# Dhole/collaborative_filtering

Measured on AMD Instinct MI355X. Metric: user-subgraph eigendecomps/sec + predicted ratings/sec, 1M users avg deg 100, higher is better.
Workload: dtype f32 (eigen) / f64 (predict)

## Files before the change

### collaborative_filtering_amd/_native.py

```python
from __future__ import annotations

import ctypes
import os
from ctypes import POINTER, c_char_p, c_double, c_float, c_int, c_int32, c_uint32, c_uint64, c_void_p

_HERE = os.path.dirname(os.path.abspath(__file__))
LIB_PATH = os.environ.get("CF_MI355X_LIB") or os.path.join(_HERE, "libcf_mi355x.so")
HOST_LIB_PATH = os.path.join(_HERE, "libcf_host.so")

CF_OK = 0
CF_EINVAL = -1
CF_ERANGE = -4
CF_ESTATE = -5
CF_KNN_SCORE_SUM = 0
CF_KNN_SCORE_MEAN = 1
CF_SVD_MAX_NV = 256
CF_ALS_MAX_D = 64
CF_TOPN_MAX_N = 1024
CF_SIGS_OWN = 0
CF_SIGS_COMPAT = 1
CF_MAX_K = 192
CF_SPILL_MAX_K = 5000
CF_EIGEN_TRIDIAG = 0
CF_EIGEN_JACOBI = 1
CF_GRAPH_DENSE = 0
CF_GRAPH_CSR = 1
CF_FILTER_CHEBY = 0
CF_FILTER_BINOMIAL = 1

SIGNATURES = {
    "cf_version": (c_int, []),
    "cf_device_count": (c_int, []),
    "cf_create": (c_int, [c_int, POINTER(c_void_p)]),
    "cf_destroy": (None, [c_void_p]),
    "cf_release_workspaces": (c_int, [c_void_p]),
    "cf_last_error": (c_char_p, [c_void_p]),
    "cf_set_jacobi": (c_int, [c_void_p, c_float, c_int]),
    "cf_set_eigen_refine": (c_int, [c_void_p, c_int, c_float, c_float]),
    "cf_set_eigen_split": (c_int, [c_void_p, c_int]),
    "cf_set_eigen_lanes": (c_int, [c_void_p, c_int]),
    "cf_debug_eigen_geometry": (c_int, [c_int, c_int, POINTER(c_int), POINTER(c_int), POINTER(c_int), POINTER(c_int),
                                        POINTER(c_int)]),
    "cf_set_pred_pack": (c_int, [c_void_p, c_int]),
    "cf_debug_split_schedule": (c_int, [c_int, c_int, POINTER(c_int), POINTER(c_int), POINTER(c_int), POINTER(c_int)]),
    "cf_set_step_masks": (c_int, [c_void_p, c_int]),
    "cf_set_local_wlim": (c_int, [c_void_p, c_int]),
    "cf_debug_predict_nmax": (c_int, [c_int]),
    "cf_set_knn2_topk": (c_int, [c_void_p, c_uint32]),
    "cf_set_eigen_method": (c_int, [c_void_p, c_int]),
    "cf_debug_stats": (c_int, [c_void_p, c_int, c_void_p]),
    "cf_eigen_bucket_timing": (c_int, [c_void_p, c_int, c_void_p]),
    "cf_eigen_bucket_timing_split": (c_int, [c_void_p, c_int, c_void_p, c_void_p]),
    "cf_debug_phases": (c_int, [c_void_p, c_int, c_void_p]),
    "cf_debug_spill": (c_int, [c_void_p, c_int, c_void_p]),
    "cf_debug_tri": (c_int, [c_void_p, c_int, c_void_p]),
    "cf_item_graph_upload": (c_int, [c_void_p, c_uint32, c_void_p, c_void_p, c_void_p]),
    "cf_item_graph_upload_dense": (c_int, [c_void_p, c_uint32, c_void_p, c_int]),
    "cf_item_graph_device": (c_void_p, [c_void_p, POINTER(c_uint32)]),
    "cf_set_graph_layout": (c_int, [c_void_p, c_int]),
    "cf_graph_info": (c_int, [c_void_p, c_void_p, c_void_p, c_void_p]),
    "cf_item_cosine_edges": (c_int, [c_void_p, c_uint32, c_uint32, c_void_p, c_void_p, c_void_p, c_float, c_int, c_int,
                                     c_void_p, c_void_p, c_void_p, c_uint64, c_void_p]),
    "cf_plan_create": (c_int, [c_void_p, c_uint32, c_void_p, POINTER(c_void_p)]),
    "cf_plan_destroy": (None, [c_void_p]),
    "cf_evec_slots": (c_uint64, [c_uint32]),
    "cf_evec_offsets": (c_uint64, [c_uint32, c_void_p, c_void_p]),
# ... 211 lines not shown
```

### collaborative_filtering_amd/api.py

```python
from __future__ import annotations

from ctypes import byref, c_double, c_float, c_int, c_uint32, c_void_p
from dataclasses import dataclass

import numpy as np

from . import _native
from ._native import CF_ERANGE, CF_FILTER_BINOMIAL, CF_FILTER_CHEBY, CF_SIGS_COMPAT, CF_SIGS_OWN, NativeError, ptr


def _check(lib, ctx, rc, what):
    if rc != _native.CF_OK:
        msg = lib.cf_last_error(ctx)
        raise NativeError(f"{what} failed ({rc}): {msg.decode() if msg else ''}")


def evec_offsets(item_off: np.ndarray) -> tuple[np.ndarray, int]:
    k = np.diff(item_off.astype(np.int64))
    slots = k * np.maximum(k, 2)
    off = np.zeros(len(k), dtype=np.uint64)
    if len(k):
        off[1:] = np.cumsum(slots)[:-1]
    return off, int(slots.sum())

# ... 279 lines not shown
            pass

    def _chk(self, rc, what):
        _check(self.lib, self.h, rc, what)

    def set_eigen_method(self, method: str = "jacobi"):
        code = {"tridiag": _native.CF_EIGEN_TRIDIAG, "jacobi": _native.CF_EIGEN_JACOBI}[method]
        self._chk(self.lib.cf_set_eigen_method(self.h, code), "cf_set_eigen_method")

    def set_jacobi(self, tol_scale: float = 1.0, max_sweeps: int = 30):
        self._chk(self.lib.cf_set_jacobi(self.h, tol_scale, max_sweeps), "cf_set_jacobi")

    def set_eigen_refine(self, enable: bool = True, stop_rel: float = 1e-3, delta: float = 1e-2):
        self._chk(self.lib.cf_set_eigen_refine(self.h, int(enable), stop_rel, delta), "cf_set_eigen_refine")

    def set_eigen_split(self, enable=True):
        self._chk(self.lib.cf_set_eigen_split(self.h, int(enable)), "cf_set_eigen_split")

    def set_eigen_lanes(self, lanes=0):
        self._chk(self.lib.cf_set_eigen_lanes(self.h, int(lanes)), "cf_set_eigen_lanes")

    def set_pred_pack(self, mode=1):
        self._chk(self.lib.cf_set_pred_pack(self.h, int(mode)), "cf_set_pred_pack")

    def set_local_wlim(self, bisect: bool = True):
        self._chk(self.lib.cf_set_local_wlim(self.h, int(bisect)), "cf_set_local_wlim")

    def set_step_masks(self, enable: bool = True):
        self._chk(self.lib.cf_set_step_masks(self.h, int(enable)), "cf_set_step_masks")

    def debug_stats(self, enable: bool = True, read: bool = False):
        out = np.zeros(8, dtype=np.uint64) if read else None
        self._chk(self.lib.cf_debug_stats(self.h, int(enable), ptr(out)), "cf_debug_stats")
        if read:
            n = max(int(out[1]), 1)
            return {"sweeps_mean": int(out[0]) / n, "users": int(out[1]), "sweeps_max": int(out[2]),
                    "capped": int(out[3]), "assembly_cyc_per_user": int(out[4]) / n,
                    "jacobi_cyc_per_user": int(out[5]) / n, "epilogue_cyc_per_user": int(out[6]) / n,
                    "jacobi_cyc_per_step": int(out[5]) / max(int(out[7]), 1)}
        return None

    def eigen_bucket_timing(self, enable: bool = True, read: bool = False, sweeps: bool = False):
        out = np.zeros(13, dtype=np.float32) if read else None
        sw = np.zeros(13, dtype=np.float32) if read else None
        self._chk(self.lib.cf_eigen_bucket_timing_split(self.h, int(enable), ptr(out), ptr(sw)),
                  "cf_eigen_bucket_timing_split")
# ... 852 lines not shown
```

### collaborative_filtering_amd/csrc/cf_api.hip

```cpp

#include <algorithm>
#include <atomic>
#include <cmath>
#include <cstring>
#include <new>

#include <type_traits>

#include "cf_internal.h"

int cf_set_error(cf_ctx* ctx, int code, const std::string& msg) {
    if (ctx) ctx->last_error = msg;
    return code;
}

namespace {
constexpr int kMaxDevices = 64;
std::atomic<int> g_ctx_per_device[kMaxDevices];
}

int cf_contexts_on_device(int device) {
    return (device >= 0 && device < kMaxDevices) ? g_ctx_per_device[device].load() : 1;
}

// ... 103 lines not shown
    drop(ctx->d_tri, ctx->tri_bytes);
    drop(ctx->d_scratch, ctx->scratch_bytes);
    drop(ctx->d_knn, ctx->knn_bytes);
    drop(ctx->d_als, ctx->als_bytes);
    return CF_OK;
}

void cf_destroy(cf_ctx* ctx) {
    if (!ctx) return;
    g_ctx_per_device[ctx->device].fetch_sub(1);
    (void)hipSetDevice(ctx->device);
    if (ctx->d_graph) (void)hipFree(ctx->d_graph);
    if (ctx->d_grp) (void)hipFree(ctx->d_grp);
    if (ctx->d_gcol) (void)hipFree(ctx->d_gcol);
    if (ctx->d_gw) (void)hipFree(ctx->d_gw);
    cf_knn_in_free(ctx);
    if (ctx->d_stats) (void)hipFree(ctx->d_stats);
    if (ctx->d_dbg) (void)hipFree(ctx->d_dbg);
    if (ctx->d_phase) (void)hipFree(ctx->d_phase);
    if (ctx->d_scratch) (void)hipFree(ctx->d_scratch);
    if (ctx->d_pred_next) (void)hipFree(ctx->d_pred_next);
    if (ctx->d_dense_q) (void)hipFree(ctx->d_dense_q);
    if (ctx->d_dense_ws) (void)hipFree(ctx->d_dense_ws);
    if (ctx->d_cmask) (void)hipFree(ctx->d_cmask);
    if (ctx->d_cmask_fp) (void)hipFree(ctx->d_cmask_fp);
    if (ctx->d_knn) (void)hipFree(ctx->d_knn);
    if (ctx->d_knn_acc) (void)hipFree(ctx->d_knn_acc);
    if (ctx->d_knn_part) (void)hipFree(ctx->d_knn_part);
    if (ctx->d_prep) (void)hipFree(ctx->d_prep);
    if (ctx->d_als) (void)hipFree(ctx->d_als);
    for (hipEvent_t& e : ctx->prep_ev)
        if (e) (void)hipEventDestroy(e);
    for (auto& run : ctx->bucket_ev)
        for (auto& pr : run)
            for (hipEvent_t& e : pr)
                if (e) (void)hipEventDestroy(e);
    if (ctx->d_spill) (void)hipFree(ctx->d_spill);
    if (ctx->d_spill_off) (void)hipFree(ctx->d_spill_off);
    if (ctx->h_spill_off) (void)hipHostFree(ctx->h_spill_off);
    if (ctx->spill_off_ev) (void)hipEventDestroy(ctx->spill_off_ev);
    for (hipEvent_t& e : ctx->spill_side_ev)
        if (e) (void)hipEventDestroy(e);
    if (ctx->spill_side) (void)hipStreamDestroy(ctx->spill_side);
    if (ctx->d_pspill) (void)hipFree(ctx->d_pspill);
    if (ctx->pspill_meta_ev) {
        (void)hipEventSynchronize(ctx->pspill_meta_ev);
// ... 578 lines not shown
```

### collaborative_filtering_amd/csrc/cf_internal.h

```cpp
#pragma once

#include <hip/hip_runtime.h>

#include <algorithm>
#include <cstdint>
#include <string>
#include <vector>

#include "cf_abi.h"

struct GraphRow {
    const float* dense;
    const uint32_t* col;
    const float* w;
    uint32_t len;
    __device__ __forceinline__ float operator[](uint32_t b) const {
        if (dense) return dense[b];
        uint32_t lo = 0, hi = len;
        while (lo < hi) {
            const uint32_t mid = (lo + hi) >> 1;
            if (col[mid] < b) lo = mid + 1;
            else hi = mid;
        }
        return (lo < len && col[lo] == b) ? w[lo] : 0.0f;
// ... 19 lines not shown
    uint32_t n_items = 0;
    int graph_layout = CF_GRAPH_DENSE;
    bool graph_csr = false;
    uint64_t* d_grp = nullptr;
    uint32_t* d_gcol = nullptr;
    float* d_gw = nullptr;
    uint64_t g_nnz = 0;
    float tol_scale = 1.0f;
    int max_sweeps = 30;
    int eigen_refine = 1;
    float stop_rel = 1e-3f;
    float refine_delta = 1e-2f;
    float close_sigrot = 8.0f;
    int eigen_sort = 2;
    unsigned long long* d_stats = nullptr;
    unsigned long long* d_phase = nullptr;
    void* d_scratch = nullptr;
    size_t scratch_bytes = 0;
    uint32_t* d_pred_next = nullptr;
    uint32_t* d_dense_q = nullptr;
    size_t dense_q_words = 0;
    double* d_dense_ws = nullptr;
    size_t dense_ws_doubles = 0;
    void* d_cmask = nullptr;
    size_t cmask_bytes = 0;
    uint64_t* d_cmask_fp = nullptr;
    uint32_t cmask_users = 0;
    uint64_t cmask_plan = 0;
    const void* cmask_key[2] = {nullptr, nullptr};
    uint64_t cmask_gen = ~0ull;
    uint64_t graph_gen = 0;
    int step_masks = 1;
    int local_wlim_bisect = 1;
    void* d_knn = nullptr;
    size_t knn_bytes = 0;
    void* d_spill = nullptr;
    size_t spill_bytes = 0;
    bool spill_debug = false;
    unsigned long long* d_dbg = nullptr;
    hipStream_t spill_side = nullptr;
    uint64_t* h_spill_off = nullptr;
    uint64_t* d_spill_off = nullptr;
    size_t spill_off_bytes = 0;
    hipEvent_t spill_off_ev = nullptr;
    hipEvent_t spill_side_ev[2] = {};
    bool spill_side_pending = false;
// ... 275 lines not shown
```

### collaborative_filtering_amd/csrc/cf_pack.hip

```cpp

#include <algorithm>
#include <thread>
#include <vector>

#include "cf_internal.h"

namespace {

constexpr int kScanThreads = 1024;

__global__ void __launch_bounds__(kScanThreads) pack_offsets_kernel(uint32_t n_users, const uint64_t* item_off,
                                                                    const int32_t* m, uint64_t* packed_off) {
    __shared__ uint64_t s_sum[kScanThreads];
    const uint32_t t = threadIdx.x;
    const uint32_t chunk = (n_users + kScanThreads - 1) / kScanThreads;
    const uint32_t u0 = min(n_users, t * chunk), u1 = min(n_users, u0 + chunk);
    uint64_t s = 0;
    for (uint32_t u = u0; u < u1; ++u) s += (item_off[u + 1] - item_off[u]) * (uint64_t)max(m[u], 0);
    s_sum[t] = s;
    __syncthreads();
    for (int d = 1; d < kScanThreads; d <<= 1) {
        const uint64_t v = t >= (uint32_t)d ? s_sum[t - d] : 0;
        __syncthreads();
        s_sum[t] += v;
        __syncthreads();
    }
    uint64_t run = s_sum[t] - s;
    for (uint32_t u = u0; u < u1; ++u) {
        packed_off[u] = run;
        run += (item_off[u + 1] - item_off[u]) * (uint64_t)max(m[u], 0);
    }
    if (t == kScanThreads - 1) packed_off[n_users] = s_sum[t];
}

__global__ void __launch_bounds__(256) pack_copy_kernel(uint32_t n_users, const uint64_t* item_off, const int32_t* m,
                                                        const uint64_t* evec_off, const float* evecs,
                                                        const uint64_t* packed_off, float* packed) {
    for (uint32_t u = blockIdx.x; u < n_users; u += gridDim.x) {
        const uint64_t n = (item_off[u + 1] - item_off[u]) * (uint64_t)max(m[u], 0);
        const float* src = evecs + evec_off[u];
        float* dst = packed + packed_off[u];
        const uint64_t mis_s = ((uintptr_t)src >> 2) & 3, mis_d = ((uintptr_t)dst >> 2) & 3;
        if (mis_s == mis_d) {
            const uint64_t head = min<uint64_t>(n, (4 - mis_s) & 3);
            for (uint64_t i = threadIdx.x; i < head; i += blockDim.x) dst[i] = src[i];
            const uint64_t nv = (n - head) / 4;
            const float4* s4 = reinterpret_cast<const float4*>(src + head);
            float4* d4 = reinterpret_cast<float4*>(dst + head);
            for (uint64_t i = threadIdx.x; i < nv; i += blockDim.x) d4[i] = s4[i];
            for (uint64_t i = head + nv * 4 + threadIdx.x; i < n; i += blockDim.x) dst[i] = src[i];
        } else {
            for (uint64_t i = threadIdx.x; i < n; i += blockDim.x) dst[i] = src[i];
        }
    }
}
// ... 58 lines not shown
        if (rcs[d] != CF_OK)
            return cf_set_error(root, rcs[d], "device part " + std::to_string(d) + ": " + ctxs[d]->last_error);
    (void)hipSetDevice(root->device);
    return CF_OK;
}

}

extern "C" {

int cf_cost_split(uint32_t n_users, const uint64_t* item_off, int n_parts, uint32_t* split) {
    if (!item_off || !split || n_parts <= 0) return CF_EINVAL;
    cost_split(n_users, item_off, n_parts, split);
    return CF_OK;
}

int cf_pack_eigen_run(cf_ctx* ctx, uint32_t n_users, const uint64_t* d_item_off, const int32_t* d_m,
                      const uint64_t* d_evec_off, const float* d_evecs, uint64_t* d_packed_off, float* d_packed,
                      void* stream) {
    if (!ctx || !d_item_off || !d_m || !d_packed_off) return cf_set_error(ctx, CF_EINVAL, "cf_pack_eigen_run: null");
    if (d_packed && (!d_evec_off || !d_evecs)) return cf_set_error(ctx, CF_EINVAL, "cf_pack_eigen_run: null evecs");
    CF_TRY(set_device(ctx));
    hipStream_t st = (hipStream_t)stream;
    hipLaunchKernelGGL(pack_offsets_kernel, dim3(1), dim3(kScanThreads), 0, st, n_users, d_item_off, d_m,
                       d_packed_off);
    CF_HIP_CHECK(ctx, hipGetLastError());
    if (d_packed && n_users) {
        const uint32_t blocks = std::min<uint32_t>(n_users, 65536u);
        hipLaunchKernelGGL(pack_copy_kernel, dim3(blocks), dim3(256), 0, st, n_users, d_item_off, d_m, d_evec_off,
                           d_evecs, (const uint64_t*)d_packed_off, d_packed);
        CF_HIP_CHECK(ctx, hipGetLastError());
    }
    return CF_OK;
}

struct multi_part {
    cf_ctx* ctx = nullptr;
    uint32_t u0 = 0, n = 0;
    uint64_t e0 = 0, ne = 0;
    uint64_t packed = 0;
    DevBuf off, items, eoff, m, sig, eval, evec, poff, pack;
    hipStream_t stream = nullptr;
    int rc = CF_OK;
};

static int multi_run_part(multi_part& p, const uint64_t* item_off, const uint32_t* items) {
    cf_ctx* ctx = p.ctx;
    CF_TRY(set_device(ctx));
    CF_HIP_CHECK(ctx, hipStreamCreateWithFlags(&p.stream, hipStreamNonBlocking));
// ... 178 lines not shown
```

### collaborative_filtering_amd/csrc/cf_predict.hip

```cpp
#include "cf_internal.h"
#include "cf_ldlt.hpp"

namespace {

constexpr int kThreads = 256;
constexpr int kWaves = kThreads / 64;
constexpr int kNsysMax = 62;
constexpr int kQuadNMax = 14;
constexpr int kPairNMax = 30;
constexpr int fast_tri(int n) { return (n + 2) * (n + 3) / 2; }
constexpr int pack_elems(int G, int nG, int lmax) { return G * (fast_tri(nG) + lmax + nG); }
constexpr double kPivMin = 1e-10;
constexpr double kOrthoMax = 1e-2;
constexpr float kOrthoDone = 1e-8f;
#ifndef CF_PRED_FS_PW
#define CF_PRED_FS_PW 8
#endif
constexpr int kFsPw = CF_PRED_FS_PW;
#ifndef CF_PRED_BASIS_OCC
#define CF_PRED_BASIS_OCC 3
#endif

struct SlotOff {
    size_t stride;
// ... 14 lines not shown
    const T* sigtab;
    int sig_mode;
    GraphDev graph;
    uint64_t n_items;
    float* mse;
    int32_t* kk;
    double* pred;
    unsigned long long* phase_cycles;
    int lmax;
    int nmax;
    int ew;
    int pack;
    int a_elems;
    int big_lds;
    int tail_basis;
    const uint64_t* cmask_in;
    uint64_t cmask_words;
    const uint64_t* cmask_fp;
    uint32_t cmask_users;
    double* slots;
    SlotOff so;
    uint32_t* dq;
    double* dense_ws;
};


template <int CTRL>
__device__ __forceinline__ double dpp_f64(double v) {
    const int lo = __builtin_amdgcn_update_dpp(0, __double2loint(v), CTRL, 0xf, 0xf, false);
    const int hi = __builtin_amdgcn_update_dpp(0, __double2hiint(v), CTRL, 0xf, 0xf, false);
    return __hiloint2double(hi, lo);
}
__device__ __forceinline__ double row16_sum(double v) {
    v += dpp_f64<0xB1>(v);
    v += dpp_f64<0x4E>(v);
    v += dpp_f64<0x141>(v);
    v += dpp_f64<0x140>(v);
    return v;
}
__device__ __forceinline__ double lane_f64(double v, int l) {
    return __hiloint2double(__builtin_amdgcn_readlane(__double2hiint(v), l), __builtin_amdgcn_readlane(__double2loint(v), l));
}
#ifdef CF_PRED_SHFL_SUM
__device__ __forceinline__ double wave_sum(double v) {
#pragma unroll
    for (int off = 32; off >= 1; off >>= 1) v += __shfl_xor(v, off);
    return v;
// ... 1368 lines not shown
                    } else {
                        wacc[5] += dt;
                    }
                }
            }
            for (int i0 = claim(&s_cnt[9], 2); i0 < n_pair; i0 = claim(&s_cnt[9], 2))
                packed(std::integral_constant<int, 2>{}, s_keep + i0, min(2, n_pair - i0));
            for (int i0 = claim(&s_cnt[10], 4); i0 < n_quad; i0 = claim(&s_cnt[10], 4))
                packed(std::integral_constant<int, 4>{}, s_nconn + i0, min(4, n_quad - i0));
            if (a.phase_cycles) {
                wacc[2] += __builtin_amdgcn_s_memtime() - fw0;
                if (lane == 0)
                    for (int x = 0; x < 8; ++x) atomicAdd(&a.phase_cycles[8 + x], wacc[x]);
            }
        }
        __syncthreads();
        const int nslow = s_cnt[7];
        if (a.phase_cycles && tid == 0) {
            ph_acc[4] += (unsigned long long)(k - nslow);
            ph_acc[5] += (unsigned long long)nslow;
        }
        PHASE_STAMP(2);

        if (a.dq && nslow > 0) {
            if (tid < nslow) {
                const int r = s_slow[tid] & 0xffff;
                const uint32_t q = atomicAdd(a.dq, 1u);
                a.dq[4 + 2 * (size_t)q] = uo;
                a.dq[4 + 2 * (size_t)q + 1] = (uint32_t)r | ((uint32_t)s_lim[r] << 16);
            }
        } else {
            for (int si = 0; si < nslow; ++si) {
                const int r = s_slow[si] & 0xffff;
                dense_rating<T>(a, r, s_lim[r], k, m, base, U, Gb, A, AP, s_item, s_rat, s_conn, s_nconn, s_keep,
                                s_cnt, s_misc);
            }
        }
        PHASE_STAMP(3);
    }
}

template <typename T>
__global__ __launch_bounds__(kThreads, CF_PRED_RATING_OCC) void pred_rating_kernel(PredArgs<T> a, uint32_t first, uint32_t count) {
    extern __shared__ double dsm[];
    unsigned long long ph_acc[8] = {0, 0, 0, 0, 0, 0, 0, 0};
    unsigned long long ph_t = 0;
    const uint32_t ub = blockIdx.x;
    if (ub < count) rating_user(a, first + ub, a.slots + (size_t)ub * a.so.stride, dsm, ph_acc, ph_t);
    if (a.phase_cycles && threadIdx.x == 0)
        for (int ph = 0; ph < 8; ++ph) atomicAdd(&a.phase_cycles[ph], ph_acc[ph]);
}

template <typename T>
__global__ __launch_bounds__(kThreads) void pred_dense_kernel(PredArgs<T> a, uint32_t first) {
    extern __shared__ double dsm[];
    double* A = dsm;
    double* s_misc = A + a.a_elems;
    double* s_gx = s_misc + 4;
    double* s_hx = s_gx + CF_MAX_K;
    uint32_t* s_item = reinterpret_cast<uint32_t*>(s_hx + CF_MAX_K);
    float* s_rat = reinterpret_cast<float*>(s_item + CF_MAX_K);
    int* s_conn = reinterpret_cast<int*>(s_rat + CF_MAX_K);
    int* s_keep = s_conn + CF_MAX_K;
    int* s_nconn = s_keep + CF_MAX_K;
    int* s_lim = s_nconn + CF_MAX_K;
    int* s_cpos = s_lim + CF_MAX_K;
    int* s_slow = s_cpos + CF_MAX_K;
    int* s_cnt = s_slow + CF_MAX_K;
    const int tid = threadIdx.x;
    double* Ahbm = a.dense_ws + (size_t)blockIdx.x * ((size_t)(a.lmax + 2) * (a.lmax + 3) / 2);
    for (;;) {
        if (tid == 0) s_cnt[8] = (int)atomicAdd(a.dq + 1, 1u);
        __syncthreads();
        const uint32_t q = (uint32_t)s_cnt[8];
        __syncthreads();
        if (q >= a.dq[0]) break;
        const uint32_t uo = a.dq[4 + 2 * (size_t)q];
        const uint32_t rl = a.dq[4 + 2 * (size_t)q + 1];
        const int r = (int)(rl & 0xffffu), lim = (int)(rl >> 16);
        const uint32_t u = a.order[uo];
        const uint64_t base = a.item_off[u];
        const int k = (int)(a.item_off[u + 1] - base);
        const int m = a.m[u];
        const T* U = a.evecs + a.evec_off[u];
        const double* Gb = a.slots + (size_t)(uo - first) * a.so.stride + a.so.gb;
        for (int i = tid; i < k; i += kThreads) {
            s_item[i] = a.items[base + i];
            s_rat[i] = a.ratings[base + i];
        }
        __syncthreads();
        dense_rating<T>(a, r, lim, k, m, base, U, Gb, A, Ahbm, s_item, s_rat, s_conn, s_nconn, s_keep, s_cnt,
                        s_misc);
    }
}

#ifdef CF_PRED_FUSED_INLINE
#define CF_PRED_CALL __forceinline__
#else
#define CF_PRED_CALL __noinline__
#endif
template <typename T>
__device__ CF_PRED_CALL void basis_user_call(const PredArgs<T> a, uint32_t uo, double* slot, double* dsm,
                                             unsigned long long (&ph_acc)[8], unsigned long long& ph_t) {
    basis_user(a, uo, slot, dsm, ph_acc, ph_t);
}
template <typename T>
__device__ CF_PRED_CALL void rating_user_call(const PredArgs<T> a, uint32_t uo, double* slot, double* dsm,
                                              unsigned long long (&ph_acc)[8], unsigned long long& ph_t) {
// ... 37 lines not shown
    so.x = (int)o; o += l2;
    so.q1 = (int)o; o += l2;
    so.ap = (int)o; o += (size_t)(lmax + 2) * (lmax + 3) / 2;
    so.gx = (int)o; o += lmax;
    so.hx = (int)o; o += lmax;
    so.misc = (int)o; o += 8;
    so.cmask = (int)o; o += 3 * (size_t)lmax;
    so.lim = (int)o; o += (lmax + 1) / 2;
    so.order = (int)o; o += (lmax + 1) / 2;
    so.cpos = (int)o; o += (lmax + 1) / 2;
    so.pmask = (int)o; o += 3 * (size_t)lmax;
    so.stride = (o + 15) & ~(size_t)15;
    return so;
}
inline size_t chunk_slot_bytes(const cf_plan* plan, uint32_t users) {
    size_t need = 0;
    for (const cf_bucket& b : plan->buckets)
        if (b.count && b.emax != kSpillBucket)
            need = std::max(need, (size_t)std::min(b.count, users) *
                                      slot_layout(std::max<int>(2, 16 * b.emax)).stride * sizeof(double));
    return need;
}
inline uint32_t fit_chunk(cf_ctx* ctx, const cf_plan* plan, size_t copies) {
    uint32_t chunk = pred_chunk();
    const size_t budget = cf_hbm_budget(ctx, ctx->scratch_bytes, 1.0 / 3.0, 0);
    while (chunk > 2048 && chunk_slot_bytes(plan, chunk) * copies > budget) chunk /= 2;
    return chunk;
}
inline int ensure_slot_scratch(cf_ctx* ctx, const cf_plan* plan, size_t copies, uint32_t& chunk) {
    for (;;) {
        const size_t need = chunk_slot_bytes(plan, chunk) * copies;
        if (need <= ctx->scratch_bytes) return CF_OK;
        if (ctx->d_scratch) (void)hipFree(ctx->d_scratch);
        ctx->d_scratch = nullptr;
        ctx->scratch_bytes = 0;
        if (hipMalloc(&ctx->d_scratch, need) == hipSuccess) {
            ctx->scratch_bytes = need;
            return CF_OK;
        }
        (void)hipGetLastError();
        ctx->d_scratch = nullptr;
        if (chunk <= 256) return cf_set_error(ctx, CF_ENOMEM, "predictor slots (" + std::to_string(need) + " bytes)");
        chunk /= 2;
    }
}
inline size_t basis_lds() {
    return sizeof(double) * (kStageElems + 4) + CF_MAX_K * (sizeof(uint32_t) + sizeof(float) + 3 * sizeof(int)) +
// ... 96 lines not shown
    args.cmask_in = cf_cmask_lookup(ctx, plan, d_item_off, d_items);
    args.cmask_words = args.cmask_in ? ctx->cmask_bytes / sizeof(uint64_t) : 0;
    args.cmask_fp = args.cmask_in ? ctx->d_cmask_fp : nullptr;
    args.cmask_users = args.cmask_in ? ctx->cmask_users : 0;
    int rc = CF_OK;
    const bool overlap = !ctx->d_phase;
    const bool fused = overlap && pred_fused_enabled();
    uint32_t fused_max = 0;
    if (fused) {
        int cus = 0;
        CF_HIP_CHECK(ctx, hipDeviceGetAttribute(&cus, hipDeviceAttributeMultiprocessorCount, ctx->device));
        fused_max = (uint32_t)std::max(1, cus) * CF_PRED_RATING_OCC;
        if (!ctx->d_pred_next)
            CF_HIP_CHECK(ctx, hipMalloc(&ctx->d_pred_next, 32 * sizeof(uint32_t) * cf_ctx::kAuxStreams));
    }
    const size_t copies = overlap ? cf_ctx::kAuxStreams : 1;
    uint32_t kChunk = fused ? fused_max : fit_chunk(ctx, plan, copies);
    CF_TRY(ensure_slot_scratch(ctx, plan, copies, kChunk));
    if (fused && kChunk != fused_max)
        return cf_set_error(ctx, CF_ENOMEM, "fused predictor slots");
    int n_cu = 0;
    CF_HIP_CHECK(ctx, hipDeviceGetAttribute(&n_cu, hipDeviceAttributeMultiprocessorCount, ctx->device));
    const uint32_t dense_grid = 2u * (uint32_t)std::max(1, n_cu);
    if (!fused) {
        const size_t qw = 4 + 2 * (size_t)kChunk * (size_t)std::max<uint32_t>(plan->kmax, 2);
        const size_t ww = (size_t)dense_grid * ((size_t)(CF_MAX_K + 2) * (CF_MAX_K + 3) / 2);
        constexpr size_t kCopies = cf_ctx::kAuxStreams;
        if (qw > ctx->dense_q_words) {
            if (ctx->d_dense_q) (void)hipFree(ctx->d_dense_q);
            ctx->d_dense_q = nullptr;
            ctx->dense_q_words = 0;
            CF_TRY(cf_malloc_evict(ctx, reinterpret_cast<void**>(&ctx->d_dense_q), sizeof(uint32_t) * qw * kCopies,
                                   "dense rating queue"));
            ctx->dense_q_words = qw;
        }
        if (ww > ctx->dense_ws_doubles) {
            if (ctx->d_dense_ws) (void)hipFree(ctx->d_dense_ws);
            ctx->d_dense_ws = nullptr;
            ctx->dense_ws_doubles = 0;
            CF_TRY(cf_malloc_evict(ctx, reinterpret_cast<void**>(&ctx->d_dense_ws), sizeof(double) * ww * kCopies,
                                   "dense factorisation regions"));
            ctx->dense_ws_doubles = ww;
        }
    }
    const size_t need = chunk_slot_bytes(plan, kChunk);
    if (fused) kChunk = 0;
    if (overlap) {
        if (!ctx->aux_stream[0]) {
            for (int i = 0; i < cf_ctx::kAuxStreams; ++i) {
                CF_HIP_CHECK(ctx, hipStreamCreateWithFlags(&ctx->aux_stream[i], hipStreamNonBlocking));
                CF_HIP_CHECK(ctx, hipEventCreateWithFlags(&ctx->aux_event[i], hipEventDisableTiming));
// ... 22 lines not shown
        if (rc != CF_OK) break;
        if (fused) {
            uint32_t grid = 0;
            size_t lds = 0;
            rc = fused_geometry<T>(ctx, rating_lds, fused_max, grid, lds);
            if (rc != CF_OK) break;
            grid = std::min(grid, b.count);
            const int si = nb++ % cf_ctx::kAuxStreams;
            hipStream_t st = ctx->aux_stream[si];
            args.slots = reinterpret_cast<double*>(static_cast<char*>(ctx->d_scratch) + si * need);
            if ((size_t)grid * args.so.stride * sizeof(double) > need) {
                rc = cf_set_error(ctx, CF_EINVAL, "predict scratch undersized");
                break;
            }
            uint32_t* next = ctx->d_pred_next + 32 * si;
            if (hipMemsetAsync(next, 0, sizeof(uint32_t), st) != hipSuccess) {
                rc = cf_set_error(ctx, CF_EHIP, "predict counter reset failed");
                break;
            }
            hipLaunchKernelGGL(pred_fused_kernel<T>, dim3(grid), dim3(kThreads), lds, st, args, b.first, b.count, next);
            if (hipGetLastError() != hipSuccess) rc = cf_set_error(ctx, CF_EHIP, "predict launch failed");
            continue;
        }
        for (uint32_t c0 = 0; c0 < b.count && rc == CF_OK; c0 += kChunk) {
            const uint32_t cnt = std::min(kChunk, b.count - c0);
            const int si = overlap ? (nb++ % cf_ctx::kAuxStreams) : 0;
            hipStream_t st = overlap ? ctx->aux_stream[si] : stream;
            args.slots = reinterpret_cast<double*>(static_cast<char*>(ctx->d_scratch) + si * need);
            if ((size_t)cnt * args.so.stride * sizeof(double) > need) {
                rc = cf_set_error(ctx, CF_EINVAL, "predict scratch undersized");
                break;
            }
            hipLaunchKernelGGL(pred_basis_kernel<T>, dim3(cnt), dim3(kThreads), basis_lds(), st, args, b.first + c0, cnt);
            args.dq = ctx->d_dense_q + si * ctx->dense_q_words;
            args.dense_ws = ctx->d_dense_ws + si * ctx->dense_ws_doubles;
            if (hipMemsetAsync(args.dq, 0, 4 * sizeof(uint32_t), st) != hipSuccess) {
                rc = cf_set_error(ctx, CF_EHIP, "dense queue reset failed");
                break;
            }
            hipLaunchKernelGGL(pred_rating_kernel<T>, dim3(cnt), dim3(kThreads), rating_lds, st, args, b.first + c0,
                               cnt);
            hipLaunchKernelGGL(pred_dense_kernel<T>, dim3(dense_grid), dim3(kThreads), rating_lds, st, args,
                               b.first + c0);
            args.dq = nullptr;
            if (hipGetLastError() != hipSuccess) rc = cf_set_error(ctx, CF_EHIP, "predict launch failed");
        }
        if (rc != CF_OK) break;
    }
    if (overlap)
        for (int i = 0; i < cf_ctx::kAuxStreams; ++i) {
            CF_HIP_CHECK(ctx, hipEventRecord(ctx->aux_event[i], ctx->aux_stream[i]));
            CF_HIP_CHECK(ctx, hipStreamWaitEvent(stream, ctx->aux_event[i], 0));
        }
    return rc;
}

int cf_launch_step(cf_ctx* ctx, const cf_plan* plan, const uint64_t* d_item_off, const uint32_t* d_items,
                   const float* d_ratings, const uint64_t* d_evec_off, int32_t* d_m, float* d_sigs, float* d_evals,
                   float* d_evecs, int sig_mode, float* d_mse, int32_t* d_kk, double* d_pred, hipStream_t stream) {
    if (ctx->eigen_method != CF_EIGEN_JACOBI || ctx->d_stats || ctx->d_phase || plan->buckets.size() > 16) {
        CF_TRY(cf_launch_eigen(ctx, plan, d_item_off, d_items, d_evec_off, d_m, d_sigs, d_evals, d_evecs, stream));
        return cf_launch_predict<float>(ctx, plan, d_item_off, d_items, d_ratings, d_m, d_evals, d_evec_off, d_evecs,
                                        d_sigs, sig_mode, d_mse, d_kk, d_pred, nullptr, stream);
    }
    if (!ctx->aux_stream[0])
        for (int i = 0; i < cf_ctx::kAuxStreams; ++i) {
            CF_HIP_CHECK(ctx, hipStreamCreateWithFlags(&ctx->aux_stream[i], hipStreamNonBlocking));
            CF_HIP_CHECK(ctx, hipEventCreateWithFlags(&ctx->aux_event[i], hipEventDisableTiming));
        }
    if (!ctx->aux_event[cf_ctx::kAuxStreams])
// ... 149 lines not shown
void cf_cmask_mark(cf_ctx* ctx, const cf_plan* plan, const uint64_t* d_item_off, const uint32_t* d_items, bool valid) {
    ctx->cmask_plan = plan->id;
    ctx->cmask_key[0] = d_item_off;
    ctx->cmask_key[1] = d_items;
    ctx->cmask_gen = valid ? ctx->graph_gen : ~0ull;
}

const uint64_t* cf_cmask_lookup(const cf_ctx* ctx, const cf_plan* plan, const uint64_t* d_item_off,
                                const uint32_t* d_items) {
    const bool hit = ctx->d_cmask && ctx->cmask_gen == ctx->graph_gen && ctx->cmask_plan == plan->id &&
                     ctx->cmask_key[0] == d_item_off && ctx->cmask_key[1] == d_items;
    return hit ? static_cast<const uint64_t*>(ctx->d_cmask) : nullptr;
}

template int cf_launch_predict<float>(cf_ctx*, const cf_plan*, const uint64_t*, const uint32_t*,
                                      const float*, const int32_t*, const float*, const uint64_t*,
                                      const float*, const float*, int, float*, int32_t*, double*,
                                      const uint8_t*, hipStream_t);
template int cf_launch_predict<double>(cf_ctx*, const cf_plan*, const uint64_t*, const uint32_t*,
                                       const float*, const int32_t*, const double*,
                                       const uint64_t*, const double*, const double*, int, float*,
                                       int32_t*, double*, const uint8_t*, hipStream_t);

extern "C" int cf_set_pred_pack(cf_ctx* ctx, int mode) {
    if (!ctx) return CF_EINVAL;
    if (mode != 0 && mode != 1) return CF_EINVAL;
    ctx->pred_pack = mode;
    return CF_OK;
}

extern "C" int cf_debug_predict_nmax(int lmax) {
    if (lmax < 2 || lmax > CF_MAX_K) return -1;
    const size_t lds_fixed = rating_lds_fixed();
    const auto per_wave = [&](int n) { return fast_tri(n) + 2 * lmax; };
    int nmax = std::min(kNsysMax, lmax);
    while (nmax > 8 && sizeof(double) * (size_t)(kWaves * per_wave(nmax)) + lds_fixed > kRatingLds) --nmax;
    return nmax;
}
```

### include/cf_abi.h

```cpp
#ifndef CF_ABI_H
#define CF_ABI_H

#include <stddef.h>
#include <stdint.h>

#ifdef __cplusplus
extern "C" {
#endif

#define CF_OK 0
#define CF_EINVAL (-1)
#define CF_ENOMEM (-2)
#define CF_EHIP (-3)
#define CF_ERANGE (-4)
#define CF_ESTATE (-5)

#define CF_MAX_K 192
#define CF_SPILL_MAX_K 5000

typedef struct cf_ctx cf_ctx;
typedef struct cf_plan cf_plan;

int cf_version(void);
int cf_device_count(void);
int cf_create(int device, cf_ctx** out);
void cf_destroy(cf_ctx* ctx);
int cf_release_workspaces(cf_ctx* ctx);
const char* cf_last_error(const cf_ctx* ctx);
#define CF_EIGEN_TRIDIAG 0
#define CF_EIGEN_JACOBI 1
int cf_set_eigen_method(cf_ctx* ctx, int method);
int cf_set_jacobi(cf_ctx* ctx, float tol_scale, int max_sweeps);
int cf_set_eigen_refine(cf_ctx* ctx, int enable, float stop_rel, float delta);
int cf_set_eigen_split(cf_ctx* ctx, int enable);
int cf_set_eigen_lanes(cf_ctx* ctx, int lanes);
int cf_debug_eigen_geometry(int emax, int lanes_setting, int* lanes, int* threads, int* ld, int* lds_bytes,
                            int* users_per_cu);
int cf_set_pred_pack(cf_ctx* ctx, int mode);
int cf_debug_split_schedule(int emax, int k, int* steps, int* levels, int* max_groups, int* max_slots);
int cf_set_step_masks(cf_ctx* ctx, int enable);
int cf_set_local_wlim(cf_ctx* ctx, int bisect);
int cf_debug_stats(cf_ctx* ctx, int enable, uint64_t* out8);
int cf_debug_spill(cf_ctx* ctx, int enable, uint64_t* out8);
int cf_debug_tri(cf_ctx* ctx, int enable, uint64_t* out8);
int cf_debug_phases(cf_ctx* ctx, int enable, uint64_t* out16);
int cf_debug_predict_nmax(int lmax);
int cf_eigen_bucket_timing(cf_ctx* ctx, int enable, float* ms13);
int cf_eigen_bucket_timing_split(cf_ctx* ctx, int enable, float* ms13, float* sweeps_ms13);

#define CF_GRAPH_DENSE 0
#define CF_GRAPH_CSR 1
int cf_set_graph_layout(cf_ctx* ctx, int layout);
int cf_graph_info(const cf_ctx* ctx, int* layout, uint32_t* n_items, uint64_t* nnz);
int cf_item_graph_upload(cf_ctx* ctx, uint32_t n_items, const uint64_t* row_ptr,
                         const uint32_t* col, const float* w);
int cf_item_graph_upload_dense(cf_ctx* ctx, uint32_t n_items, const float* w_dense,
                               int on_device);
const float* cf_item_graph_device(const cf_ctx* ctx, uint32_t* n_items);

int cf_plan_create(cf_ctx* ctx, uint32_t n_users, const uint64_t* item_off, cf_plan** out);
void cf_plan_destroy(cf_plan* plan);
// ... 306 lines not shown
```

Baseline: 350,700.

## Parallelize pack offset scan and add deferred dense-rating stream path

Replaces the single-block pack offset scan with a three-kernel multi-block scan: per-block wave-shuffle scan, a carry pass, then an add pass. Adds an optional deferred dense-rating mode. In that mode slow rows are queued with a copied Gbar into a pool and processed by a dense kernel on a separate stream joined by events. The goal is to overlap dense work with the basis and rating kernels. The deferred mode is gated by an env var and setters and is off by default. The scan change always runs and adds extra launches and a block-sum buffer.

```diff
diff --git a/collaborative_filtering_amd/_native.py b/collaborative_filtering_amd/_native.py
--- a/collaborative_filtering_amd/_native.py
+++ b/collaborative_filtering_amd/_native.py
@@ -42,6 +42,10 @@
     "cf_debug_eigen_geometry": (c_int, [c_int, c_int, POINTER(c_int), POINTER(c_int), POINTER(c_int), POINTER(c_int),
                                         POINTER(c_int)]),
     "cf_set_pred_pack": (c_int, [c_void_p, c_int]),
+    "cf_set_pred_dense": (c_int, [c_void_p, c_int]),
+    "cf_set_pred_dense_pool": (c_int, [c_void_p, c_int]),
+    "cf_set_pred_chunk": (c_int, [c_void_p, c_uint32]),
+    "cf_debug_pred_dense": (c_int, [c_void_p, c_void_p]),
     "cf_debug_split_schedule": (c_int, [c_int, c_int, POINTER(c_int), POINTER(c_int), POINTER(c_int), POINTER(c_int)]),
     "cf_set_step_masks": (c_int, [c_void_p, c_int]),
     "cf_set_local_wlim": (c_int, [c_void_p, c_int]),
diff --git a/collaborative_filtering_amd/api.py b/collaborative_filtering_amd/api.py
--- a/collaborative_filtering_amd/api.py
+++ b/collaborative_filtering_amd/api.py
@@ -325,6 +325,20 @@
 
     def set_pred_pack(self, mode=1):
         self._chk(self.lib.cf_set_pred_pack(self.h, int(mode)), "cf_set_pred_pack")
+
+    def set_pred_dense(self, mode=0):
+        self._chk(self.lib.cf_set_pred_dense(self.h, int(mode)), "cf_set_pred_dense")
+
+    def set_pred_dense_pool(self, entries=-1):
+        self._chk(self.lib.cf_set_pred_dense_pool(self.h, int(entries)), "cf_set_pred_dense_pool")
+
+    def set_pred_chunk(self, users=0):
+        self._chk(self.lib.cf_set_pred_chunk(self.h, int(users)), "cf_set_pred_chunk")
+
+    def debug_pred_dense(self):
+        out = np.zeros(4, dtype=np.uint32)
+        self._chk(self.lib.cf_debug_pred_dense(self.h, ptr(out)), "cf_debug_pred_dense")
+        return {"pool_users": int(out[0]), "queued": int(out[1]), "own_users": int(out[2])}
 
     def set_local_wlim(self, bisect: bool = True):
         self._chk(self.lib.cf_set_local_wlim(self.h, int(bisect)), "cf_set_local_wlim")
diff --git a/collaborative_filtering_amd/csrc/cf_api.hip b/collaborative_filtering_amd/csrc/cf_api.hip
--- a/collaborative_filtering_amd/csrc/cf_api.hip
+++ b/collaborative_filtering_amd/csrc/cf_api.hip
@@ -149,6 +149,12 @@
     if (ctx->d_pred_next) (void)hipFree(ctx->d_pred_next);
     if (ctx->d_dense_q) (void)hipFree(ctx->d_dense_q);
     if (ctx->d_dense_ws) (void)hipFree(ctx->d_dense_ws);
+    if (ctx->d_pack_sum) (void)hipFree(ctx->d_pack_sum);
+    if (ctx->d_dd_hdr) (void)hipFree(ctx->d_dd_hdr);
+    if (ctx->d_dd_pool) (void)hipFree(ctx->d_dd_pool);
+    for (hipEvent_t& e : ctx->dense_event)
+        if (e) (void)hipEventDestroy(e);
+    if (ctx->dense_stream) (void)hipStreamDestroy(ctx->dense_stream);
     if (ctx->d_cmask) (void)hipFree(ctx->d_cmask);
     if (ctx->d_cmask_fp) (void)hipFree(ctx->d_cmask_fp);
     if (ctx->d_knn) (void)hipFree(ctx->d_knn);
diff --git a/collaborative_filtering_amd/csrc/cf_internal.h b/collaborative_filtering_amd/csrc/cf_internal.h
--- a/collaborative_filtering_amd/csrc/cf_internal.h
+++ b/collaborative_filtering_amd/csrc/cf_internal.h
@@ -65,6 +65,19 @@
     size_t dense_q_words = 0;
     double* d_dense_ws = nullptr;
     size_t dense_ws_doubles = 0;
+    uint64_t* d_pack_sum = nullptr;
+    size_t pack_sum_words = 0;
+    static constexpr int kDenseHdrWords = 64;
+    static constexpr uint32_t kDenseQCap = 8192;
+    static constexpr uint32_t kDensePoolCap = 1024;
+    uint32_t* d_dd_hdr = nullptr;
+    double* d_dd_pool = nullptr;
+    size_t dd_pool_doubles = 0;
+    hipStream_t dense_stream = nullptr;
+    hipEvent_t dense_event[3] = {};
+    int pred_dense = -1;
+    int pred_dense_pool = -1;
+    uint32_t pred_chunk = 0;
     void* d_cmask = nullptr;
     size_t cmask_bytes = 0;
     uint64_t* d_cmask_fp = nullptr;
diff --git a/collaborative_filtering_amd/csrc/cf_pack.hip b/collaborative_filtering_amd/csrc/cf_pack.hip
--- a/collaborative_filtering_amd/csrc/cf_pack.hip
+++ b/collaborative_filtering_amd/csrc/cf_pack.hip
@@ -8,29 +8,60 @@
 namespace {
 
 constexpr int kScanThreads = 1024;
+constexpr uint32_t kScanCarryMax = kScanThreads;
+
+__device__ __forceinline__ uint64_t pack_block_scan(uint64_t v, uint64_t* s_wave, uint64_t& total) {
+    const int lane = threadIdx.x & 63, wave = threadIdx.x >> 6;
+    uint64_t inc = v;
+#pragma unroll
+    for (int d = 1; d < 64; d <<= 1) {
+        const uint64_t o = (uint64_t)__shfl_up((unsigned long long)inc, d);
+        if (lane >= d) inc += o;
+    }
+    if (lane == 63) s_wave[wave] = inc;
+    __syncthreads();
+    uint64_t before = 0;
+    total = 0;
+    for (int w = 0; w < kScanThreads / 64; ++w) {
+        const uint64_t sw = s_wave[w];
+        if (w < wave) before += sw;
+        total += sw;
+    }
+    __syncthreads();
+    return before + inc - v;
+}
 
 __global__ void __launch_bounds__(kScanThreads) pack_offsets_kernel(uint32_t n_users, const uint64_t* item_off,
-                                                                    const int32_t* m, uint64_t* packed_off) {
-    __shared__ uint64_t s_sum[kScanThreads];
-    const uint32_t t = threadIdx.x;
-    const uint32_t chunk = (n_users + kScanThreads - 1) / kScanThreads;
-    const uint32_t u0 = min(n_users, t * chunk), u1 = min(n_users, u0 + chunk);
-    uint64_t s = 0;
-    for (uint32_t u = u0; u < u1; ++u) s += (item_off[u + 1] - item_off[u]) * (uint64_t)max(m[u], 0);
-    s_sum[t] = s;
-    __syncthreads();
-    for (int d = 1; d < kScanThreads; d <<= 1) {
-        const uint64_t v = t >= (uint32_t)d ? s_sum[t - d] : 0;
-        __syncthreads();
-        s_sum[t] += v;
-        __syncthreads();
-    }
-    uint64_t run = s_sum[t] - s;
-    for (uint32_t u = u0; u < u1; ++u) {
-        packed_off[u] = run;
-        run += (item_off[u + 1] - item_off[u]) * (uint64_t)max(m[u], 0);
-    }
-    if (t == kScanThreads - 1) packed_off[n_users] = s_sum[t];
+                                                                    const int32_t* m, uint64_t* packed_off,
+                                                                    uint64_t* block_sum) {
+    __shared__ uint64_t s_wave[kScanThreads / 64];
+    const uint64_t u = (uint64_t)blockIdx.x * kScanThreads + threadIdx.x;
+    const uint64_t v = u < n_users ? (item_off[u + 1] - item_off[u]) * (uint64_t)max(m[u], 0) : 0;
+    uint64_t total;
+    const uint64_t ex = pack_block_scan(v, s_wave, total);
+    if (u < n_users) packed_off[u] = ex;
+    if (threadIdx.x == 0) block_sum[blockIdx.x] = total;
+}
+
+__global__ void __launch_bounds__(kScanThreads) pack_carry_kernel(uint32_t n_blocks, uint64_t* block_sum,
+                                                                  uint64_t* total_out) {
+    __shared__ uint64_t s_wave[kScanThreads / 64];
+    uint64_t carry = 0;
+    for (uint32_t b0 = 0; b0 < n_blocks; b0 += kScanCarryMax) {
+        const uint32_t b = b0 + threadIdx.x;
+        const uint64_t v = b < n_blocks ? block_sum[b] : 0;
+        uint64_t total;
+        const uint64_t ex = pack_block_scan(v, s_wave, total);
+        if (b < n_blocks) block_sum[b] = carry + ex;
+        carry += total;
+    }
+    if (threadIdx.x == 0) *total_out = carry;
+}
+
+__global__ void __launch_bounds__(kScanThreads) pack_offsets_add_kernel(uint32_t n_users, const uint64_t* block_sum,
+                                                                        uint64_t* packed_off) {
+    const uint64_t u = (uint64_t)blockIdx.x * kScanThreads + threadIdx.x;
+    if (u < n_users) packed_off[u] += block_sum[blockIdx.x];
 }
 
 __global__ void __launch_bounds__(256) pack_copy_kernel(uint32_t n_users, const uint64_t* item_off, const int32_t* m,
@@ -135,9 +166,29 @@
     if (d_packed && (!d_evec_off || !d_evecs)) return cf_set_error(ctx, CF_EINVAL, "cf_pack_eigen_run: null evecs");
     CF_TRY(set_device(ctx));
     hipStream_t st = (hipStream_t)stream;
-    hipLaunchKernelGGL(pack_offsets_kernel, dim3(1), dim3(kScanThreads), 0, st, n_users, d_item_off, d_m,
-                       d_packed_off);
+    const uint32_t n_blocks = (uint32_t)(((uint64_t)n_users + kScanThreads - 1) / kScanThreads);
+    if (std::max<size_t>(n_blocks, 1) > ctx->pack_sum_words) {
+        if (ctx->d_pack_sum) (void)hipFree(ctx->d_pack_sum);
+        ctx->d_pack_sum = nullptr;
+        ctx->pack_sum_words = 0;
+        const size_t words = std::max<size_t>(n_blocks, 1024);
+        CF_TRY(cf_malloc_evict(ctx, reinterpret_cast<void**>(&ctx->d_pack_sum), sizeof(uint64_t) * words,
+                               "pack block sums"));
+        ctx->pack_sum_words = words;
+    }
+    if (n_blocks) {
+        hipLaunchKernelGGL(pack_offsets_kernel, dim3(n_blocks), dim3(kScanThreads), 0, st, n_users, d_item_off, d_m,
+                           d_packed_off, ctx->d_pack_sum);
+        CF_HIP_CHECK(ctx, hipGetLastError());
+    }
+    hipLaunchKernelGGL(pack_carry_kernel, dim3(1), dim3(kScanThreads), 0, st, n_blocks, ctx->d_pack_sum,
+                       d_packed_off + n_users);
     CF_HIP_CHECK(ctx, hipGetLastError());
+    if (n_blocks > 1) {
+        hipLaunchKernelGGL(pack_offsets_add_kernel, dim3(n_blocks), dim3(kScanThreads), 0, st, n_users,
+                           (const uint64_t*)ctx->d_pack_sum, d_packed_off);
+        CF_HIP_CHECK(ctx, hipGetLastError());
+    }
     if (d_packed && n_users) {
         const uint32_t blocks = std::min<uint32_t>(n_users, 65536u);
         hipLaunchKernelGGL(pack_copy_kernel, dim3(blocks), dim3(256), 0, st, n_users, d_item_off, d_m, d_evec_off,
diff --git a/collaborative_filtering_amd/csrc/cf_predict.hip b/collaborative_filtering_amd/csrc/cf_predict.hip
--- a/collaborative_filtering_amd/csrc/cf_predict.hip
+++ b/collaborative_filtering_amd/csrc/cf_predict.hip
@@ -60,7 +60,14 @@
     SlotOff so;
     uint32_t* dq;
     double* dense_ws;
+    uint32_t* dd_hdr;
+    uint32_t* dd_cnt;
+    uint32_t* dd_ent;
+    double* dd_pool;
+    size_t dd_pstride;
+    uint32_t dd_qcap, dd_pcap;
 };
+constexpr uint32_t kDenseVoid = 0xffffffffu;
 
 
 template <int CTRL>
@@ -1475,14 +1482,47 @@
         }
         PHASE_STAMP(2);
 
-        if (a.dq && nslow > 0) {
+        bool queued = false;
+        if (a.dd_hdr && nslow > 0) {
+            if (tid == 0) {
+                const uint32_t pe = a.dd_hdr[0] < a.dd_pcap ? atomicAdd(&a.dd_hdr[0], 1u) : a.dd_pcap;
+                s_cnt[9] = pe < a.dd_pcap;
+                s_cnt[10] = (int)pe;
+                if (pe < a.dd_pcap) s_cnt[8] = (int)atomicAdd(&a.dd_cnt[0], (uint32_t)nslow);
+            }
+            __syncthreads();
+            const bool have = s_cnt[9] != 0;
+            const uint32_t q0 = (uint32_t)s_cnt[8], pe = (uint32_t)s_cnt[10];
+            queued = have && (uint64_t)q0 + (uint64_t)nslow <= (uint64_t)a.dd_qcap;
+            if (have && tid < nslow && (uint64_t)q0 + (uint64_t)tid < (uint64_t)a.dd_qcap) {
+                const int r = s_slow[tid] & 0xffff;
+                uint32_t* ent = a.dd_ent + 3 * ((size_t)q0 + tid);
+                ent[0] = queued ? uo : kDenseVoid;
+                ent[1] = (uint32_t)r | ((uint32_t)s_lim[r] << 16);
+                ent[2] = pe;
+            }
+            if (queued) {
+                double* dst = a.dd_pool + (size_t)pe * a.dd_pstride;
+                for (int i = tid; i < lmax * lmax; i += kThreads) dst[i] = Gb[i];
+                __threadfence();
+                __syncthreads();
+                if (tid == 0) {
+                    atomicAdd(&a.dd_hdr[1], (uint32_t)nslow);
+                    atomicAdd(&a.dd_hdr[3], 1u);
+                }
+            } else if (tid == 0) {
+                atomicAdd(&a.dd_hdr[2], 1u);
+            }
+        } else if (a.dq && nslow > 0) {
+            queued = true;
             if (tid < nslow) {
                 const int r = s_slow[tid] & 0xffff;
                 const uint32_t q = atomicAdd(a.dq, 1u);
                 a.dq[4 + 2 * (size_t)q] = uo;
                 a.dq[4 + 2 * (size_t)q + 1] = (uint32_t)r | ((uint32_t)s_lim[r] << 16);
             }
-        } else {
+        }
+        if (!queued) {
             for (int si = 0; si < nslow; ++si) {
                 const int r = s_slow[si] & 0xffff;
                 dense_rating<T>(a, r, s_lim[r], k, m, base, U, Gb, A, AP, s_item, s_rat, s_conn, s_nconn, s_keep,
@@ -1522,21 +1562,26 @@
     int* s_cnt = s_slow + CF_MAX_K;
     const int tid = threadIdx.x;
     double* Ahbm = a.dense_ws + (size_t)blockIdx.x * ((size_t)(a.lmax + 2) * (a.lmax + 3) / 2);
+    uint32_t* cnt = a.dd_hdr ? a.dd_cnt : a.dq;
+    const uint32_t n_q = a.dd_hdr ? min(cnt[0], a.dd_qcap) : cnt[0];
     for (;;) {
-        if (tid == 0) s_cnt[8] = (int)atomicAdd(a.dq + 1, 1u);
+        if (tid == 0) s_cnt[8] = (int)atomicAdd(cnt + 1, 1u);
         __syncthreads();
         const uint32_t q = (uint32_t)s_cnt[8];
         __syncthreads();
-        if (q >= a.dq[0]) break;
-        const uint32_t uo = a.dq[4 + 2 * (size_t)q];
-        const uint32_t rl = a.dq[4 + 2 * (size_t)q + 1];
+        if (q >= n_q) break;
+        const uint32_t* ent = a.dd_hdr ? a.dd_ent + 3 * (size_t)q : a.dq + 4 + 2 * (size_t)q;
+        const uint32_t uo = ent[0];
+        const uint32_t rl = ent[1];
+        if (uo == kDenseVoid) continue;
         const int r = (int)(rl & 0xffffu), lim = (int)(rl >> 16);
         const uint32_t u = a.order[uo];
         const uint64_t base = a.item_off[u];
         const int k = (int)(a.item_off[u + 1] - base);
         const int m = a.m[u];
         const T* U = a.evecs + a.evec_off[u];
-        const double* Gb = a.slots + (size_t)(uo - first) * a.so.stride + a.so.gb;
+        const double* Gb = a.dd_hdr ? a.dd_pool + (size_t)ent[2] * a.dd_pstride
+                                    : a.slots + (size_t)(uo - first) * a.so.stride + a.so.gb;
         for (int i = tid; i < k; i += kThreads) {
             s_item[i] = a.items[base + i];
             s_rat[i] = a.ratings[base + i];
@@ -1620,7 +1665,7 @@
     return need;
 }
 inline uint32_t fit_chunk(cf_ctx* ctx, const cf_plan* plan, size_t copies) {
-    uint32_t chunk = pred_chunk();
+    uint32_t chunk = ctx->pred_chunk ? ctx->pred_chunk : pred_chunk();
     const size_t budget = cf_hbm_budget(ctx, ctx->scratch_bytes, 1.0 / 3.0, 0);
     while (chunk > 2048 && chunk_slot_bytes(plan, chunk) * copies > budget) chunk /= 2;
     return chunk;
@@ -1763,11 +1808,43 @@
     int n_cu = 0;
     CF_HIP_CHECK(ctx, hipDeviceGetAttribute(&n_cu, hipDeviceAttributeMultiprocessorCount, ctx->device));
     const uint32_t dense_grid = 2u * (uint32_t)std::max(1, n_cu);
+    if (ctx->pred_dense < 0) {
+        const char* e = std::getenv("CF_PRED_DENSE");
+        ctx->pred_dense = e && e[0] == '1' ? 1 : e && e[0] == '2' ? 2 : 0;
+    }
+    const bool deferred = overlap && !fused && ctx->pred_dense != 0;
+    const uint32_t pool_cap = ctx->pred_dense == 2 ? 0u
+                              : ctx->pred_dense_pool >= 0 ? (uint32_t)ctx->pred_dense_pool : cf_ctx::kDensePoolCap;
+    constexpr size_t kSegWords = 3 * (size_t)cf_ctx::kDenseQCap;
+    size_t pool_stride = 0;
+    if (deferred) {
+        for (const cf_bucket& b : plan->buckets)
+            if (b.count && b.emax != kSpillBucket) {
+                const size_t l = (size_t)std::max<int>(2, 16 * b.emax);
+                pool_stride = std::max(pool_stride, l * l);
+            }
+        if (!ctx->d_dd_hdr)
+            CF_TRY(cf_malloc_evict(ctx, reinterpret_cast<void**>(&ctx->d_dd_hdr),
+                                   sizeof(uint32_t) * (cf_ctx::kDenseHdrWords + 13 * kSegWords), "dense rating queue"));
+        const size_t pw = pool_stride * pool_cap;
+        if (pw > ctx->dd_pool_doubles) {
+            if (ctx->d_dd_pool) (void)hipFree(ctx->d_dd_pool);
+            ctx->d_dd_pool = nullptr;
+            ctx->dd_pool_doubles = 0;
+            CF_TRY(cf_malloc_evict(ctx, reinterpret_cast<void**>(&ctx->d_dd_pool), sizeof(double) * pw, "dense Gbar pool"));
+            ctx->dd_pool_doubles = pw;
+        }
+        if (!ctx->dense_stream) {
+            CF_HIP_CHECK(ctx, hipStreamCreateWithFlags(&ctx->dense_stream, hipStreamNonBlocking));
+            for (hipEvent_t& e : ctx->dense_event) CF_HIP_CHECK(ctx, hipEventCreateWithFlags(&e, hipEventDisableTiming));
+        }
+        CF_HIP_CHECK(ctx, hipMemsetAsync(ctx->d_dd_hdr, 0, sizeof(uint32_t) * cf_ctx::kDenseHdrWords, stream));
+    }
     if (!fused) {
         const size_t qw = 4 + 2 * (size_t)kChunk * (size_t)std::max<uint32_t>(plan->kmax, 2);
         const size_t ww = (size_t)dense_grid * ((size_t)(CF_MAX_K + 2) * (CF_MAX_K + 3) / 2);
         constexpr size_t kCopies = cf_ctx::kAuxStreams;
-        if (qw > ctx->dense_q_words) {
+        if (!deferred && qw > ctx->dense_q_words) {
             if (ctx->d_dense_q) (void)hipFree(ctx->d_dense_q);
             ctx->d_dense_q = nullptr;
             ctx->dense_q_words = 0;
@@ -1836,6 +1913,16 @@
             if (hipGetLastError() != hipSuccess) rc = cf_set_error(ctx, CF_EHIP, "predict launch failed");
             continue;
         }
+        if (deferred) {
+            args.dd_hdr = ctx->d_dd_hdr;
+            args.dd_cnt = ctx->d_dd_hdr + 4 + 2 * b.emax;
+            args.dd_ent = ctx->d_dd_hdr + cf_ctx::kDenseHdrWords + (size_t)b.emax * kSegWords;
+            args.dd_qcap = cf_ctx::kDenseQCap;
+            args.dd_pool = ctx->d_dd_pool;
+            args.dd_pstride = pool_stride;
+            args.dd_pcap = pool_cap;
+            args.dense_ws = ctx->d_dense_ws;
+        }
         for (uint32_t c0 = 0; c0 < b.count && rc == CF_OK; c0 += kChunk) {
             const uint32_t cnt = std::min(kChunk, b.count - c0);
             const int si = overlap ? (nb++ % cf_ctx::kAuxStreams) : 0;
@@ -1846,6 +1933,12 @@
                 break;
             }
             hipLaunchKernelGGL(pred_basis_kernel<T>, dim3(cnt), dim3(kThreads), basis_lds(), st, args, b.first + c0, cnt);
+            if (deferred) {
+                hipLaunchKernelGGL(pred_rating_kernel<T>, dim3(cnt), dim3(kThreads), rating_lds, st, args, b.first + c0,
+                                   cnt);
+                if (hipGetLastError() != hipSuccess) rc = cf_set_error(ctx, CF_EHIP, "predict launch failed");
+                continue;
+            }
             args.dq = ctx->d_dense_q + si * ctx->dense_q_words;
             args.dense_ws = ctx->d_dense_ws + si * ctx->dense_ws_doubles;
             if (hipMemsetAsync(args.dq, 0, 4 * sizeof(uint32_t), st) != hipSuccess) {
@@ -1860,6 +1953,27 @@
             if (hipGetLastError() != hipSuccess) rc = cf_set_error(ctx, CF_EHIP, "predict launch failed");
         }
         if (rc != CF_OK) break;
+        if (deferred) {
+            hipError_t e = hipSuccess;
+            for (int i = 0; i < cf_ctx::kAuxStreams && e == hipSuccess; ++i) {
+                e = hipEventRecord(ctx->dense_event[i], ctx->aux_stream[i]);
+                if (e == hipSuccess) e = hipStreamWaitEvent(ctx->dense_stream, ctx->dense_event[i], 0);
+            }
+            if (e == hipSuccess) {
+                hipLaunchKernelGGL(pred_dense_kernel<T>, dim3(dense_grid), dim3(kThreads), rating_lds, ctx->dense_stream,
+                                   args, b.first);
+                e = hipGetLastError();
+            }
+            if (e != hipSuccess) {
+                rc = cf_set_error(ctx, CF_EHIP, std::string("dense launch: ") + hipGetErrorString(e));
+                break;
+            }
+        }
+    }
+    if (deferred) {
+        hipError_t e = hipEventRecord(ctx->dense_event[cf_ctx::kAuxStreams], ctx->dense_stream);
+        if (e == hipSuccess) e = hipStreamWaitEvent(stream, ctx->dense_event[cf_ctx::kAuxStreams], 0);
+        if (e != hipSuccess && rc == CF_OK) rc = cf_set_error(ctx, CF_EHIP, std::string("dense join: ") + hipGetErrorString(e));
     }
     if (overlap)
         for (int i = 0; i < cf_ctx::kAuxStreams; ++i) {
@@ -2055,6 +2169,38 @@
                                        const uint64_t*, const double*, const double*, int, float*,
                                        int32_t*, double*, const uint8_t*, hipStream_t);
 
+extern "C" int cf_set_pred_dense(cf_ctx* ctx, int mode) {
+    if (!ctx) return CF_EINVAL;
+    if (mode < 0 || mode > 2) return CF_EINVAL;
+    ctx->pred_dense = mode;
+    return CF_OK;
+}
+
+extern "C" int cf_set_pred_dense_pool(cf_ctx* ctx, int entries) {
+    if (!ctx) return CF_EINVAL;
+    if (entries < -1 || entries > (1 << 20)) return CF_EINVAL;
+    ctx->pred_dense_pool = entries;
+    return CF_OK;
+}
+
+extern "C" int cf_set_pred_chunk(cf_ctx* ctx, uint32_t users) {
+    if (!ctx) return CF_EINVAL;
+    if (users > (1u << 20)) return CF_EINVAL;
+    ctx->pred_chunk = users;
+    return CF_OK;
+}
+
+extern "C" int cf_debug_pred_dense(cf_ctx* ctx, uint32_t* out4) {
+    if (!ctx || !out4) return CF_EINVAL;
+    CF_TRY(set_device(ctx));
+    std::fill(out4, out4 + 4, 0u);
+    if (!ctx->d_dd_hdr) return CF_OK;
+    CF_HIP_CHECK(ctx, hipDeviceSynchronize());
+    CF_HIP_CHECK(ctx, hipMemcpy(out4, ctx->d_dd_hdr, 4 * sizeof(uint32_t), hipMemcpyDeviceToHost));
+    std::swap(out4[0], out4[3]);
+    return CF_OK;
+}
+
 extern "C" int cf_set_pred_pack(cf_ctx* ctx, int mode) {
     if (!ctx) return CF_EINVAL;
     if (mode != 0 && mode != 1) return CF_EINVAL;
diff --git a/include/cf_abi.h b/include/cf_abi.h
--- a/include/cf_abi.h
+++ b/include/cf_abi.h
@@ -37,6 +37,10 @@
 int cf_debug_eigen_geometry(int emax, int lanes_setting, int* lanes, int* threads, int* ld, int* lds_bytes,
                             int* users_per_cu);
 int cf_set_pred_pack(cf_ctx* ctx, int mode);
+int cf_set_pred_dense(cf_ctx* ctx, int mode);
+int cf_set_pred_dense_pool(cf_ctx* ctx, int entries);
+int cf_set_pred_chunk(cf_ctx* ctx, uint32_t users);
+int cf_debug_pred_dense(cf_ctx* ctx, uint32_t* out4);
 int cf_debug_split_schedule(int emax, int k, int* steps, int* levels, int* max_groups, int* max_slots);
 int cf_set_step_masks(cf_ctx* ctx, int enable);
 int cf_set_local_wlim(cf_ctx* ctx, int bisect);
```

Result: no change. 351,300, median of 6 (+0.2%).
